# NVlabs/nvdiffrecmc

Measured on NVIDIA H100. Metric: shadow_rays_per_second_train_step, higher is better.
Workload: dtype f32

## Files before the change

include/mcshade.h:

```cpp
#ifndef MCSHADE_H
#define MCSHADE_H
#include <stdint.h>

#ifdef __cplusplus
extern "C" {
#endif

#define MCS_ABI_VERSION 2

typedef struct mcs_tensor {
    const void *ptr;
    int32_t sizes[4];
    int32_t strides[4];
} mcs_tensor;

typedef struct mcs_ctx mcs_ctx;
typedef void *mcs_stream;

int mcs_abi_version(void);
const char *mcs_last_error(void);

int mcs_ctx_create(mcs_ctx **out);
int mcs_ctx_destroy(mcs_ctx *ctx);

int mcs_bvh_build(mcs_ctx *ctx, const float *verts, int32_t V, const int32_t *tris, int32_t T, uint32_t rebuild, mcs_stream stream);

int mcs_bvh_export(mcs_ctx *ctx, uint32_t *morton, int32_t *prim, int32_t *left, int32_t *right, float *lo, float *hi, mcs_stream stream);

int mcs_trace_visibility(mcs_ctx *ctx, const float *ro, const float *rd, int64_t n, uint8_t *vis, mcs_stream stream);

int mcs_trace_closest(mcs_ctx *ctx, const float *ro, const float *rd, int64_t n, int32_t *tri_id, float *tuv, mcs_stream stream);

int mcs_env_shade_fwd(mcs_ctx *ctx,
                      const mcs_tensor *mask, const mcs_tensor *ro, const mcs_tensor *gb_pos, const mcs_tensor *gb_normal,
                      const mcs_tensor *gb_view_pos, const mcs_tensor *gb_kd, const mcs_tensor *gb_ks,
                      const mcs_tensor *light, const mcs_tensor *pdf, const mcs_tensor *rows, const mcs_tensor *cols,
                      const mcs_tensor *perms,
                      uint32_t bsdf, uint32_t n_samples_x, uint32_t rnd_seed, const uint32_t *seed_offset_dev, float shadow_scale, int32_t batch_offset,
                      float *diff, float *spec, uint32_t *hit_record, uint32_t *rec_count, float *rec_rays, int32_t rec_slots, mcs_stream stream);

int mcs_env_shade_bwd(mcs_ctx *ctx,
                      const mcs_tensor *mask, const mcs_tensor *ro, const mcs_tensor *gb_pos, const mcs_tensor *gb_normal,
// ... 101 lines not shown
```

nvdiffrecmc_b200/_lib.py:

```python
import collections
import ctypes as C
import os
import subprocess
import sys
from concurrent.futures import ThreadPoolExecutor

_PKG = os.path.dirname(os.path.abspath(__file__))
_CSRC = os.path.join(_PKG, "csrc")
_LIBDIR = os.path.join(_PKG, "lib")
LIB_PATH = os.environ.get("MCS_LIB", os.path.join(_LIBDIR, "libmcshade.so"))
SOURCES = ["core.cu", "elementwise.cu", "denoise.cu", "bvh.cu", "envshade.cu", "lossmesh.cu", "light.cu", "raster.cu"]
NVCC_FLAGS = ["-O3", "-std=c++17", "-gencode", "arch=compute_90a,code=sm_90a", "-lineinfo", "-Xcompiler", "-fPIC"]


def _nvcc():
    for cand in (os.environ.get("CUDA_HOME", "") + "/bin/nvcc", "/usr/local/cuda/bin/nvcc", "nvcc"):
        if cand and (os.path.isabs(cand) and os.path.exists(cand)):
            return cand
    return "nvcc"


def build(force=False, verbose=False):
    os.makedirs(_LIBDIR, exist_ok=True)
    objdir = os.path.join(_LIBDIR, "obj")
# ... 31 lines not shown

class mcs_tensor(C.Structure):
    _fields_ = [("ptr", C.c_void_p), ("sizes", C.c_int32 * 4), ("strides", C.c_int32 * 4)]


_lib = None
_T = C.POINTER(mcs_tensor)
_P = C.c_void_p
_SIGS = {
    "mcs_abi_version": ([], C.c_int),
    "mcs_last_error": ([], C.c_char_p),
    "mcs_ctx_create": ([C.POINTER(_P)], C.c_int),
    "mcs_ctx_destroy": ([_P], C.c_int),
    "mcs_bvh_build": ([_P, _P, C.c_int32, _P, C.c_int32, C.c_uint32, _P], C.c_int),
    "mcs_bvh_export": ([_P] * 8, C.c_int),
    "mcs_trace_visibility": ([_P, _P, _P, C.c_int64, _P, _P], C.c_int),
    "mcs_trace_closest": ([_P, _P, _P, C.c_int64, _P, _P, _P], C.c_int),
    "mcs_env_shade_fwd": ([_P] + [_T] * 12 + [C.c_uint32, C.c_uint32, C.c_uint32, _P, C.c_float, C.c_int32, _P, _P, _P, _P, _P, C.c_int32, _P], C.c_int),
    "mcs_env_shade_bwd_replay": ([_T] * 6 + [C.c_uint32, C.c_uint32, C.c_float, _T, _T, _P, _P, C.c_int32] + [_P] * 6, C.c_int),
    "mcs_env_shade_records": ([_P] + [_T] * 12 + [C.c_uint32, C.c_uint32, C.c_uint32, _P, C.c_float, C.c_int32, _P, _P, _P, _P, _P], C.c_int),
    "mcs_env_shade_bwd": ([_P] + [_T] * 12 + [C.c_uint32, C.c_uint32, C.c_uint32, _P, C.c_float, C.c_int32, _T, _T] + [_P] * 7, C.c_int),
    "mcs_bilateral_fwd": ([_T, _T, _T, C.c_float, _P, _P], C.c_int),
    "mcs_bilateral_bwd": ([_T, _T, C.c_float, _T, _P, _P], C.c_int),
    "mcs_bilateral_fwd2": ([_T, _T, _T, _T, C.c_float, _P, _P, _P], C.c_int),
    "mcs_bilateral_bwd2": ([_T, _T, C.c_float, _T, _T, _P, _P, _P], C.c_int),
    "mcs_lambert_fwd": ([_T] * 2 + [_P] * 2, C.c_int),
    "mcs_lambert_bwd": ([_T] * 3 + [_P] * 3, C.c_int),
    "mcs_frostbite_fwd": ([_T] * 4 + [_P] * 2, C.c_int),
    "mcs_frostbite_bwd": ([_T] * 5 + [_P] * 5, C.c_int),
    "mcs_fresnel_shlick_fwd": ([_T] * 3 + [_P] * 2, C.c_int),
# ... 41 lines not shown
        raise RuntimeError(
            "libmcshade.so not found at %s -- build it with `python -c 'import __graft_entry__ as g; g.build()'` "
            "(nvcc, sm_90a). There is no CPU / PyTorch fallback for the hot path." % LIB_PATH)
    l = C.CDLL(LIB_PATH)
    for name, (args, res) in _SIGS.items():
        fn = getattr(l, name)
        fn.argtypes = args
        fn.restype = res
    if l.mcs_abi_version() != 2:
        raise RuntimeError("libmcshade ABI version mismatch")
    _lib = l
    return l


LAUNCHES = collections.Counter()
_KERNELS_PER_CALL = {"optix_build_bvh": 11, "bvh_export": 0, "update_pdf": 2, "rasterize": 2, "antialias_topology": 2}


def check(status, what):
    LAUNCHES[what] += _KERNELS_PER_CALL.get(what, 1)
    if status != 0:
        msg = lib().mcs_last_error()
        raise RuntimeError("%s failed (status %d): %s" % (what, status, msg.decode() if msg else "?"))


def _desc(ptr, sizes, strides):
    t = mcs_tensor()
    t.ptr = ptr
    for i in range(4):
        t.sizes[i] = int(sizes[i])
        t.strides[i] = int(strides[i])
# ... 45 lines not shown
```

nvdiffrecmc_b200/csrc/bvh.cu:

```cuda
#include "bvh_traverse.cuh"
#include "ctx.h"

int mcs_buf_reserve(DevBuf &b, size_t bytes, cudaStream_t s)
{
    if (bytes <= b.cap) return 0;
    size_t ncap = b.cap ? b.cap : 256;
    while (ncap < bytes) ncap *= 2;
    if (b.p) MCS_CUDA(cudaFreeAsync(b.p, s));
    b.p = nullptr; b.cap = 0;
    MCS_CUDA(cudaMallocAsync(&b.p, ncap, s));
    b.cap = ncap;
    return 0;
}

namespace {

__device__ __forceinline__ uint32_t f2ord(float f) { uint32_t b = __float_as_uint(f); return (b & 0x80000000u) ? ~b : (b | 0x80000000u); }
__device__ __forceinline__ float ord2f(uint32_t u) { return __uint_as_float((u & 0x80000000u) ? (u & 0x7FFFFFFFu) : ~u); }

__global__ void k_bounds_init(uint32_t *bounds)
{
    int i = threadIdx.x;
    if (i < 12) bounds[i] = ((i / 3) & 1) ? 0u : 0xFFFFFFFFu;
}
// ... 303 lines not shown
            nodes[1] = make_float4(INFINITY, -INFINITY, INFINITY, -INFINITY);
            nodes[2] = make_float4(lo[2], hi[2], INFINITY, -INFINITY);
            nodes[3] = make_float4(__int_as_float(~((0 << 3) | (T - 1))), __int_as_float(~0), 0.0f, 0.0f);
        }
        return;
    }
    if (i >= T - 1) return;
    int c0 = left[i], c1 = right[i];
    const float *l0 = lo + 3 * (size_t)c0, *h0 = hi + 3 * (size_t)c0, *l1 = lo + 3 * (size_t)c1, *h1 = hi + 3 * (size_t)c1;
    nodes[4 * (size_t)i + 0] = make_float4(l0[0], h0[0], l0[1], h0[1]);
    nodes[4 * (size_t)i + 1] = make_float4(l1[0], h1[0], l1[1], h1[1]);
    nodes[4 * (size_t)i + 2] = make_float4(l0[2], h0[2], l1[2], h1[2]);
    nodes[4 * (size_t)i + 3] = make_float4(__int_as_float(child_code(c0, T, range)), __int_as_float(child_code(c1, T, range)), 0.0f, 0.0f);
}

__device__ __forceinline__ void emit_nodeq(const int i, int T, const int32_t *left, const int32_t *right, const int2 *range, const float *lo, const float *hi,
                                           uint4 *nodesq4, float *qgrid)
{
    float org[3], inv_cell[3];
#pragma unroll
    for (int a = 0; a < 3; ++a) {
        org[a] = lo[a];
        const float ext = __fsub_rn(hi[a], lo[a]);
        int e;
        const float m = frexpf(fmaxf(ext, 1e-30f) * (1.0f / 65532.0f), &e);
        const int k = (m == 0.5f) ? e - 1 : e;
        inv_cell[a] = ldexpf(1.0f, -k);
        if (i == 0) { qgrid[a] = org[a]; qgrid[3 + a] = ldexpf(1.0f, k); qgrid[6 + a] = inv_cell[a]; }
    }
    const bool tiny = T <= MCS_LEAF_MAX;
    if (tiny ? i != 0 : i >= T - 1) return;
    int cn[2], code[2];
    if (tiny) { cn[0] = 0; cn[1] = -1; code[0] = ~((0 << 3) | (T - 1)); code[1] = ~0; }
    else { cn[0] = left[i]; cn[1] = right[i]; code[0] = child_code(cn[0], T, range); code[1] = child_code(cn[1], T, range); }
    int gn[4] = {-1, -1, -1, -1}, gcode[4] = {~0, ~0, ~0, ~0}, ng = 0;
#pragma unroll
    for (int c = 0; c < 2; ++c) {
        if (cn[c] < 0) continue;
        if (code[c] < 0) { gn[ng] = cn[c]; gcode[ng] = code[c]; ++ng; }
        else {
            const int g0 = left[cn[c]], g1 = right[cn[c]];
            gn[ng] = g0; gcode[ng] = child_code(g0, T, range); ++ng;
            gn[ng] = g1; gcode[ng] = child_code(g1, T, range); ++ng;
        }
    }
    uint32_t leaf_bits = 0u;
#pragma unroll
    for (int c = 0; c < 4; ++c) leaf_bits |= (gcode[c] < 0 ? 1u : 0u) << c;
#pragma unroll
    for (int c = 0; c < 4; ++c) {
        uint32_t ql[3] = {65535u, 65535u, 65535u}, qh[3] = {0u, 0u, 0u};
        if (gn[c] >= 0) {
#pragma unroll
            for (int a = 0; a < 3; ++a) {
                const float fl = floorf(__fmul_rn(__fsub_rn(lo[3 * (size_t)gn[c] + a], org[a]), inv_cell[a])) - 2.0f;
                const float fh = ceilf(__fmul_rn(__fsub_rn(hi[3 * (size_t)gn[c] + a], org[a]), inv_cell[a])) + 2.0f;
                ql[a] = (uint32_t)fminf(fmaxf(fl, 0.0f), 65535.0f);
                qh[a] = (uint32_t)fminf(fmaxf(fh, 0.0f), 65535.0f);
            }
        }
        const uint32_t payload = (uint32_t)(gcode[c] < 0 ? ~gcode[c] : gcode[c]) & 0x0FFFFFFFu;
        nodesq4[4 * (size_t)i + c] = make_uint4(ql[0] | (qh[0] << 16), ql[1] | (qh[1] << 16), ql[2] | (qh[2] << 16), payload | (c == 0 ? leaf_bits << 28 : 0u));
    }
}

__global__ void __launch_bounds__(256) k_emit_both(int T, const int32_t *left, const int32_t *right, const int2 *range, const float *lo, const float *hi,
                                                   float4 *nodes, uint4 *nodesq4, float *qgrid)
{
    const int i = blockIdx.x * blockDim.x + threadIdx.x;
    emit_node(i, T, left, right, range, lo, hi, nodes);
    emit_nodeq(i, T, left, right, range, lo, hi, nodesq4, qgrid);
}

typedef BvhView VisView;
__global__ void __launch_bounds__(128) k_visibility(VisView b, const float *__restrict__ ro, const float *__restrict__ rd, int64_t n, uint8_t *__restrict__ vis)
{
    int64_t i = (int64_t)blockIdx.x * blockDim.x + threadIdx.x;
    if (i >= n) return;
    f3 o = F3(ro[3 * i], ro[3 * i + 1], ro[3 * i + 2]), d = F3(rd[3 * i], rd[3 * i + 1], rd[3 * i + 2]);
    vis[i] = bvh_occluded(b, o, d) ? 0 : 1;
}

__global__ void __launch_bounds__(128) k_closest(BvhView b, const float *__restrict__ ro, const float *__restrict__ rd, int64_t n,
                                                 int32_t *__restrict__ tri_id, float *__restrict__ tuv)
{
    int64_t i = (int64_t)blockIdx.x * blockDim.x + threadIdx.x;
// ... 14 lines not shown
{
    MCS_REQUIRE(out != nullptr, "mcs_ctx_create: null output pointer");
    int dev = 0;
    MCS_CUDA(cudaGetDevice(&dev));
    mcs_ctx *c = new mcs_ctx();
    c->device = dev;
    *out = c;
    return 0;
}

int mcs_ctx_destroy(mcs_ctx *c)
{
    if (!c) return 0;
    DevBuf *bufs[] = {&c->bounds, &c->tlo, &c->thi, &c->keys, &c->keys_alt, &c->vals, &c->vals_alt, &c->left, &c->right, &c->parent,
                      &c->lo, &c->hi, &c->flags, &c->range, &c->sort_tmp, &c->nodes, &c->tris, &c->nodesq4, &c->qgrid, &c->lcg_skip[0], &c->lcg_skip[1], &c->lcg_skip[2], &c->lcg_skip[3],
                      &c->counters, &c->mtx_inv};
    for (DevBuf *b : bufs)
        if (b->p) cudaFree(b->p);
    delete c;
    return 0;
}

int mcs_bvh_build(mcs_ctx *c, const float *verts, int32_t V, const int32_t *tris, int32_t T, uint32_t rebuild, mcs_stream stream)
{
    cudaStream_t s = (cudaStream_t)stream;
    MCS_REQUIRE(c != nullptr, "mcs_bvh_build: null context");
    MCS_REQUIRE(verts && tris, "mcs_bvh_build: null geometry pointer");
    MCS_REQUIRE(T > 0 && V > 0, "Got empty training triangle mesh (unrecoverable discontinuity)");
    MCS_REQUIRE(T <= (1 << 25), "mcs_bvh_build: at most 2^25 triangles (28-bit child words of the quantised nodes), got %d", T);
    MCS_REQUIRE(rebuild != 0 || c->T == T, "mcs_bvh_build: refit (rebuild=0) needs an existing structure with the same triangle count (have %d, got %d)", c->T, T);
    const size_t nT = (size_t)T, nN = 2 * nT - 1;
// ... 24 lines not shown
    if (rebuild) {
        k_morton<<<nblk(T, 256), 256, 0, s>>>(tlo, thi, T, bounds, (uint32_t *)c->keys_alt.p, (int32_t *)c->vals_alt.p);
        MCS_LAUNCH_CHECK();
        if (int e = rs_sort_pairs((uint32_t *)c->keys_alt.p, (int32_t *)c->vals_alt.p, (uint32_t *)c->keys.p, (int32_t *)c->vals.p, T, c->sort_tmp, s)) return e;
        if (T > 1) {
            k_karras<<<nblk(T - 1, 256), 256, 0, s>>>((const uint32_t *)c->keys_alt.p, T, (int32_t *)c->left.p, (int32_t *)c->right.p, (int32_t *)c->parent.p,
                                                      (int2 *)c->range.p);
            MCS_LAUNCH_CHECK();
        }
    }
    MCS_CUDA(cudaMemsetAsync(c->flags.p, 0, nT * sizeof(int), s));
    k_leaves_refit<<<nblk(T, REFIT_THREADS), REFIT_THREADS, 0, s>>>(verts, tris, T, tlo, thi, (const int32_t *)c->vals_alt.p, bounds, (const int32_t *)c->left.p,
                                                                   (const int32_t *)c->right.p, (const int32_t *)c->parent.p, (const int2 *)c->range.p,
                                                                   (float *)c->lo.p, (float *)c->hi.p, (int *)c->flags.p, (float4 *)c->tris.p);
    MCS_LAUNCH_CHECK();
    k_emit_both<<<nblk(T > 1 ? T - 1 : 1, 256), 256, 0, s>>>(T, (const int32_t *)c->left.p, (const int32_t *)c->right.p, (const int2 *)c->range.p,
                                                              (const float *)c->lo.p, (const float *)c->hi.p, (float4 *)c->nodes.p, (uint4 *)c->nodesq4.p,
                                                              (float *)c->qgrid.p);
    MCS_LAUNCH_CHECK();
    c->T = T; c->V = V;
    return 0;
}

int mcs_bvh_export(mcs_ctx *c, uint32_t *morton, int32_t *prim, int32_t *left, int32_t *right, float *lo, float *hi, mcs_stream stream)
{
    cudaStream_t s = (cudaStream_t)stream;
    MCS_REQUIRE(c && c->T > 0, "mcs_bvh_export: no acceleration structure built");
    size_t T = (size_t)c->T;
    MCS_CUDA(cudaMemcpyAsync(morton, c->keys_alt.p, T * sizeof(uint32_t), cudaMemcpyDeviceToDevice, s));
    MCS_CUDA(cudaMemcpyAsync(prim, c->vals_alt.p, T * sizeof(int32_t), cudaMemcpyDeviceToDevice, s));
    if (T > 1) {
        MCS_CUDA(cudaMemcpyAsync(left, c->left.p, (T - 1) * sizeof(int32_t), cudaMemcpyDeviceToDevice, s));
        MCS_CUDA(cudaMemcpyAsync(right, c->right.p, (T - 1) * sizeof(int32_t), cudaMemcpyDeviceToDevice, s));
    }
    MCS_CUDA(cudaMemcpyAsync(lo, c->lo.p, (2 * T - 1) * 3 * sizeof(float), cudaMemcpyDeviceToDevice, s));
    MCS_CUDA(cudaMemcpyAsync(hi, c->hi.p, (2 * T - 1) * 3 * sizeof(float), cudaMemcpyDeviceToDevice, s));
    return 0;
}

int mcs_trace_visibility(mcs_ctx *c, const float *ro, const float *rd, int64_t n, uint8_t *vis, mcs_stream stream)
{
    MCS_REQUIRE(c && c->T > 0, "mcs_trace_visibility: no acceleration structure built (call mcs_bvh_build first)");
    MCS_REQUIRE(n >= 0 && (n == 0 || (ro && rd && vis)), "mcs_trace_visibility: bad arguments");
    if (n == 0) return 0;
    VisView b{(const float4 *)c->nodes.p, (const float4 *)c->tris.p, nullptr, nullptr};
    k_visibility<<<nblk(n, 128), 128, 0, (cudaStream_t)stream>>>(b, ro, rd, n, vis);
    MCS_LAUNCH_CHECK();
    return 0;
}

int mcs_trace_closest(mcs_ctx *c, const float *ro, const float *rd, int64_t n, int32_t *tri_id, float *tuv, mcs_stream stream)
{
    MCS_REQUIRE(c && c->T > 0, "mcs_trace_closest: no acceleration structure built (call mcs_bvh_build first)");
    MCS_REQUIRE(n >= 0 && (n == 0 || (ro && rd && tri_id && tuv)), "mcs_trace_closest: bad arguments");
// ... 9 lines not shown
```

nvdiffrecmc_b200/csrc/ctx.h:

```cpp
#pragma once
#include "common.cuh"

#define MCS_SKIP_TABLES 4
#define MCS_COUNTER_RING 64

struct DevBuf {
    void *p = nullptr;
    size_t cap = 0;
};

struct mcs_ctx {
    int device = 0;
    int T = 0, V = 0;
    DevBuf bounds;
    DevBuf tlo, thi;
    DevBuf keys, keys_alt;
    DevBuf vals, vals_alt;
    DevBuf left, right, parent;
    DevBuf lo, hi;
    DevBuf flags;
    DevBuf range;
    DevBuf sort_tmp;
    DevBuf nodes;
    DevBuf tris;
    DevBuf nodesq4;
    DevBuf qgrid;
    DevBuf lcg_skip[MCS_SKIP_TABLES];
    int skip_N[MCS_SKIP_TABLES] = {0, 0, 0, 0};
    int n_skip = 0;
    unsigned skip_evict = 0;
    DevBuf counters;
    unsigned counter_next = 0;
    DevBuf mtx_inv;
};

int mcs_buf_reserve(DevBuf &b, size_t bytes, cudaStream_t s);
```

nvdiffrecmc_b200/csrc/envshade.cu:

```cuda
#include "bsdf.cuh"
#include "bvh_traverse.cuh"
#include "ctx.h"
#include "exact.cuh"
#include <vector>

namespace {

constexpr float MIN_ROUGHNESS = 0.08f;

struct EnvParams {
    TView mask, ro, pos, nrm, view, kd, ks;
    const float *light; int l_s1, l_s2, l_s3;
    const float *pdf; int p_s1, p_s2;
    const float *rows; int r_s;
    const float *cols; int c_s1, c_s2;
    const int32_t *perms; int pm_s1, pm_s3; uint32_t n_perms;
    int Hl, Wl, m_rows, m_cols;
    int B, H, W;
    int N, S;
    uint32_t bsdf, seed;
    const uint32_t *seed_dev;
    int batch_offset;
    float shadow_scale;
    BvhView bvh;
// ... 195 lines not shown
#ifndef MCS_SPLIT_WALKS
#define MCS_SPLIT_WALKS 1
#endif
#ifndef MCS_SPLIT_BELOW
#define MCS_SPLIT_BELOW 20
#endif
#ifndef MCS_QSTACK
#define MCS_QSTACK 100
#endif
#ifndef MCS_LEAF_BATCH
#define MCS_LEAF_BATCH 32
#endif
#ifndef MCS_REFILL_BELOW
#define MCS_REFILL_BELOW 24
#endif
constexpr int NW = MCS_CTA_WARPS;
constexpr int SEG = 128;
constexpr int QTOT = NW * SEG;
#ifndef MCS_PCAP
#define MCS_PCAP 160
#endif
constexpr int PCAP = MCS_PCAP;
constexpr int PIXRING = 256;
static_assert(QTOT <= 65536, "queue entry index is stored in 16 bits");
static_assert(SEG <= 256 && SEG % 32 == 0, "sample slot within a fill is stored in 8 bits");

struct BlockQueue {
    float dx[QTOT], dy[QTOT], dz[QTOT], mis[QTOT];
    uint32_t tex[QTOT];
    uint16_t vlist[QTOT];
// ... 184 lines not shown

__device__ __forceinline__ void trace_queue(const EnvParams &p, BlockQueue &q, const int warp, const int lane)
{
    constexpr int REFILL_BELOW = MCS_REFILL_BELOW;
    constexpr int LEAF_BATCH = MCS_LEAF_BATCH;
    unsigned lt;
    asm("mov.u32 %0, %%lanemask_lt;" : "=r"(lt));
    int pend = 0;
    int my = -1;
    int node = 0, sp = 0, sb = 0;
    int stack[MCS_QSTACK];
    RayQ r; r.ax = r.ay = r.az = 1.0f; r.bx = r.by = r.bz = 0.0f; r.nx = r.ny = r.nz = 0x7410u; r.fx = r.fy = r.fz = 0x7432u;
    const BvhView b = p.bvh;
    uint2 *pl = q.pl[warp];
    int seg = warp, exhausted = 0;

    auto leaf_batch = [&](int n) {
        __syncwarp();
        const int base = pend - n;
        if (lane < n) {
            const uint2 ent = pl[base + lane];
            const int e = (int)ent.x;
            if (!(q.tex[e] >> 31)) {
                const int code = (int)ent.y;
                const int start = code >> 3, cnt = (code & 7) + 1;
                const int ps = e / SEG;
                const f3 o = F3(q.ro[ps][0], q.ro[ps][1], q.ro[ps][2]);
                const f3 d = F3(q.dx[e], q.dy[e], q.dz[e]);
                bool hit = false;
                for (int k = 0; k < cnt && !hit; ++k) {
                    const float4 *t = b.tris + 3 * (size_t)(start + k);
                    const float4 t0 = __ldg(t), t1 = __ldg(t + 1), t2 = __ldg(t + 2);
                    float tt, uu, vv;
                    hit = mt_hit(o, d, F3(t0.x, t0.y, t0.z), F3(t1.x, t1.y, t1.z), F3(t2.x, t2.y, t2.z), MCS_TMAX, tt, uu, vv);
                }
                if (hit) atomicOr(&q.tex[e], 0x80000000u);
            }
        }
        pend = base;
        __syncwarp();
    };

    while (true) {
        unsigned idle = __ballot_sync(0xFFFFFFFFu, my < 0);
        while (idle && exhausted < NW) {
            const int need = __popc(idle);
            int base = 0;
            if (lane == 0) base = atomicAdd(&q.seg_head[seg], need);
            base = __shfl_sync(0xFFFFFFFFu, base, 0);
            const int avail = q.seg_cnt[seg] - base;
            if (avail <= 0) { seg = seg + 1 == NW ? 0 : seg + 1; ++exhausted; continue; }
            const int take = avail < need ? avail : need;
            const int rank = __popc(idle & lt);
            if (my < 0 && rank < take) {
                const int idx = seg * SEG + base + rank;
                my = idx;
                r = rayq_fetch(b.qgrid, q.rog[seg], q.dx[idx], q.dy[idx], q.dz[idx]);
                node = 0; sp = 0; sb = 0;
            }
            if (take < need) { seg = seg + 1 == NW ? 0 : seg + 1; ++exhausted; }
            idle = __ballot_sync(0xFFFFFFFFu, my < 0);
        }
#if MCS_SPLIT_WALKS
        if (exhausted >= NW && idle) {
            const unsigned donors = __ballot_sync(0xFFFFFFFFu, my >= 0 && sp > sb);
            if (donors) {
                const int npair = min(__popc(idle), __popc(donors));
                uint2 *xch = pl + (PCAP - 32);
                const int kd = __popc(donors & lt), ki = __popc(idle & lt);
                if (my >= 0 && sp > sb && kd < npair) { xch[kd] = make_uint2((unsigned)my, (unsigned)stack[sb]); ++sb; }
                __syncwarp();
                if (my < 0 && ki < npair) {
                    const uint2 g = xch[ki];
// ... 5 lines not shown
            }
        }
#endif
        int nact = __popc(__ballot_sync(0xFFFFFFFFu, my >= 0));
        if (nact == 0) {
            if (pend == 0) break;
            leaf_batch(pend < 32 ? pend : 32);
            continue;
        }
        const int thresh = exhausted < NW ? REFILL_BELOW : (MCS_SPLIT_WALKS ? MCS_SPLIT_BELOW : 1);
        do {
            const int cur = my;
            unsigned lmask = 0u;
            int c0 = 0, c1 = 0, c2 = 0, c3 = 0;
            if (my >= 0) {
                const uint4 *n = b.nodesq4 + 4 * (size_t)node;
                const uint4 k0 = __ldg(n), k1 = __ldg(n + 1), k2 = __ldg(n + 2), k3 = __ldg(n + 3);
                const bool h0 = qslab(k0, r), h1 = qslab(k1, r), h2 = qslab(k2, r), h3 = qslab(k3, r);
                const unsigned hm = (h0 ? 1u : 0u) | (h1 ? 2u : 0u) | (h2 ? 4u : 0u) | (h3 ? 8u : 0u);
                const unsigned lb = k0.w >> 28;
                c0 = (int)(k0.w & 0x0FFFFFFFu); c1 = (int)k1.w; c2 = (int)k2.w; c3 = (int)k3.w;
                lmask = hm & lb;
                const unsigned im = hm & ~lb;
                stack[sp] = c0; sp += (int)(im & 1u);
                stack[sp] = c1; sp += (int)((im >> 1) & 1u);
                stack[sp] = c2; sp += (int)((im >> 2) & 1u);
                stack[sp] = c3; sp += (int)(im >> 3);
                if (im) { node = (im & 8u) ? c3 : ((im & 4u) ? c2 : ((im & 2u) ? c1 : c0)); --sp; }
                else if (sp > sb) node = stack[--sp];
                else my = -1;
// ... 1 lines not shown
            for (unsigned mL = __ballot_sync(0xFFFFFFFFu, lmask != 0u); mL; mL = __ballot_sync(0xFFFFFFFFu, lmask != 0u)) {
                if (lmask) {
                    const unsigned low = lmask & (0u - lmask);
                    const int code = (low & 3u) ? ((low & 1u) ? c0 : c1) : ((low & 4u) ? c2 : c3);
                    pl[pend + __popc(mL & lt)] = make_uint2((unsigned)cur, (unsigned)code);
                    lmask ^= low;
                }
                pend += __popc(mL);
                if (PCAP < 160 && pend >= LEAF_BATCH) leaf_batch(32);
            }
            nact = __popc(__ballot_sync(0xFFFFFFFFu, my >= 0));
        } while (pend < LEAF_BATCH && nact >= thresh);
        while (pend >= LEAF_BATCH) leaf_batch(32);
        if (my >= 0 && (q.tex[my] >> 31)) my = -1;
    }
    __syncwarp();
}

template <int MODE>
__global__ void __launch_bounds__(NW * 32, 32 / NW) env_shade_kernel(const EnvParams p)
{
    extern __shared__ __align__(16) unsigned char smem_raw[];
    const int lane = threadIdx.x & 31, warp = threadIdx.x >> 5;
    BlockQueue &q = *reinterpret_cast<BlockQueue *>(smem_raw);
    BlockQueueRec *qr = MODE == 2 ? reinterpret_cast<BlockQueueRec *>(smem_raw + sizeof(BlockQueue)) : nullptr;

    const int64_t npix = (int64_t)p.B * p.H * p.W;
    const unsigned int nchunks = (unsigned int)((npix + 31) / 32);
    const int S = p.S, items = 2 * S;
    const float sample_frac = (xf(1.0f) / xf((float)(unsigned)(p.N * p.N))).v;
// ... 342 lines not shown
    p.Hl = light->sizes[1]; p.Wl = light->sizes[2];
    MCS_REQUIRE(light->sizes[3] == 3 && p.Hl >= 2 && p.Wl >= 2, "env_shade: light must be [Hl>=2, Wl>=2, 3]");
    MCS_REQUIRE(p.Hl < 32768 && p.Wl < 65536, "env_shade: light probe too large");
    MCS_REQUIRE(pdf->sizes[1] == p.Hl && pdf->sizes[2] == p.Wl && cols->sizes[1] == p.Hl && cols->sizes[2] == p.Wl && rows->sizes[1] == p.Hl,
                "env_shade: pdf / rows / cols do not match the light probe resolution");
    p.light = (const float *)light->ptr; p.l_s1 = light->strides[1]; p.l_s2 = light->strides[2]; p.l_s3 = light->strides[3];
    p.pdf = (const float *)pdf->ptr; p.p_s1 = pdf->strides[1]; p.p_s2 = pdf->strides[2];
    p.rows = (const float *)rows->ptr; p.r_s = rows->strides[1];
    p.cols = (const float *)cols->ptr; p.c_s1 = cols->strides[1]; p.c_s2 = cols->strides[2];
    p.N = (int)n_samples_x; p.S = p.N * p.N;
    p.hit_words = (2 * p.S + 31) / 32;
    MCS_REQUIRE(perms->sizes[3] == p.S && perms->sizes[1] >= 1, "env_shade: perms must be [P, n_samples_x^2]");
    p.perms = (const int32_t *)perms->ptr; p.pm_s1 = perms->strides[1]; p.pm_s3 = perms->strides[3]; p.n_perms = (uint32_t)perms->sizes[1];
    p.m_rows = cdf_iters(p.Hl); p.m_cols = cdf_iters(p.Wl);
    p.bsdf = bsdf; p.seed = rnd_seed; p.seed_dev = seed_offset_dev; p.batch_offset = batch_offset; p.shadow_scale = shadow_scale;
    p.bvh = BvhView{(const float4 *)ctx->nodes.p, (const float4 *)ctx->tris.p, (const float *)ctx->qgrid.p, (const uint4 *)ctx->nodesq4.p};
    if (int e = ensure_skip_table(ctx, p.N, s, &p.skip)) return e;
    if (int e = mcs_buf_reserve(ctx->counters, MCS_COUNTER_RING * 64, s)) return e;
    p.chunk_counter = (unsigned int *)((char *)ctx->counters.p + 64 * (size_t)(ctx->counter_next++ % MCS_COUNTER_RING));
    MCS_CUDA(cudaMemsetAsync(p.chunk_counter, 0, sizeof(unsigned int), s));
    return 0;
}

template <int MODE>
static int launch_env(const EnvParams &p, cudaStream_t s)
{
    int dev = 0, sms = 0, per_sm = 0;
    MCS_CUDA(cudaGetDevice(&dev));
    MCS_CUDA(cudaDeviceGetAttribute(&sms, cudaDevAttrMultiProcessorCount, dev));
    const size_t smem = sizeof(BlockQueue) + (MODE == 2 ? sizeof(BlockQueueRec) : 0);
    MCS_CUDA(cudaFuncSetAttribute(env_shade_kernel<MODE>, cudaFuncAttributeMaxDynamicSharedMemorySize, (int)smem));
// ... 101 lines not shown
    p.sample_frac = 1.0f / (float)(n_samples_x * n_samples_x);
    p.pos_grad = gb_pos_grad; p.nrm_grad = gb_normal_grad; p.kd_grad = gb_kd_grad; p.ks_grad = gb_ks_grad; p.light_grad = light_grad;
    MCS_CUDA(cudaMemsetAsync(light_grad, 0, sizeof(float) * 3 * (size_t)p.Hl * p.Wl, s));
    int dev = 0, sms = 0;
    MCS_CUDA(cudaGetDevice(&dev));
    MCS_CUDA(cudaDeviceGetAttribute(&sms, cudaDevAttrMultiProcessorCount, dev));
    const int64_t npix = (int64_t)p.B * p.H * p.W;
    int64_t want = (npix + 255) / 256;
    int grid = (int)(want < (int64_t)sms * 8 ? want : (int64_t)sms * 8);
    if (grid < 1) grid = 1;
    env_shade_replay_kernel<<<grid, 256, 0, s>>>(p);
    MCS_LAUNCH_CHECK();
    return 0;
}

}
```

nvdiffrecmc_b200/optixutils/ops.py:

```python
import ctypes as C

import numpy as np
import torch

from .. import _lib as L

_BSDF_MODES = ['pbr', 'diffuse', 'white']
HIT_RECORD_REPLAY = "rays"
RAY_RECORD_MAX_BYTES = 32 << 30
RAY_RECORD_MAX_FREE_FRACTION = 0.5


_fits_cache = {}


def _ray_record_fits(nbytes, device):
    if nbytes > RAY_RECORD_MAX_BYTES:
        return False
    key = (str(device), int(nbytes))
    if torch.cuda.is_current_stream_capturing():
        return _fits_cache.get(key, True)
    _fits_cache[key] = _ray_record_fits_now(nbytes, device)
    return _fits_cache[key]

# ... 186 lines not shown
                                      L.stream_ptr()), "trace_closest")
    return tid, tuv


def bvh_export(optix_ctx):
    T = optix_ctx._geom[1].shape[0]
    dev = optix_ctx._geom[0].device
    morton = torch.empty(T, dtype=torch.int32, device=dev); prim = torch.empty(T, dtype=torch.int32, device=dev)
    left = torch.empty(max(T - 1, 1), dtype=torch.int32, device=dev); right = torch.empty(max(T - 1, 1), dtype=torch.int32, device=dev)
    lo = torch.empty(2 * T - 1, 3, dtype=torch.float32, device=dev); hi = torch.empty(2 * T - 1, 3, dtype=torch.float32, device=dev)
    L.check(L.lib().mcs_bvh_export(optix_ctx.cpp_wrapper, morton.data_ptr(), prim.data_ptr(), left.data_ptr(), right.data_ptr(), lo.data_ptr(),
                                   hi.data_ptr(), L.stream_ptr()), "bvh_export")
    return dict(morton=morton, prim=prim, left=left[:T - 1], right=right[:T - 1], lo=lo, hi=hi)


class _bilateral_denoiser_func(torch.autograd.Function):
    @staticmethod
    def forward(ctx, col, nrm, zdz, sigma):
        L.require_cuda(col, nrm, zdz)
        ctx.save_for_backward(nrm, zdz)
        ctx.sigma = sigma
        B, H, W = col.shape[0], col.shape[1], col.shape[2]
        out = torch.empty(B, H, W, 4, dtype=torch.float32, device=col.device)
        c, n, z = L.nhwc(_f32(col, "col")), L.nhwc(_f32(nrm, "nrm")), L.nhwc(_f32(zdz, "zdz"))
        L.check(L.lib().mcs_bilateral_fwd(C.byref(c), C.byref(n), C.byref(z), float(sigma), out.data_ptr(), L.stream_ptr()), "bilateral_denoiser (forward)")
        return out

    @staticmethod
    def backward(ctx, out_grad):
        nrm, zdz = ctx.saved_tensors
# ... 81 lines not shown
```

Baseline: 5341.

## Build SAH-aware PLOC BVH with multi-triangle leaves for shadow traversal

For meshes up to a size limit, adds a single-block PLOC agglomerative clustering pass that builds a binary BVH with SAH-based leaf collapsing (up to 8 triangles per leaf). It then emits a 4-wide quantized node array and reorders triangles so leaves are contiguous. The shadow-ray tracer in the shading kernel uses these reordered triangles, aiming to reduce node visits and triangle tests compared with the LBVH. The cost is two extra kernels per BVH build, and k_ploc runs on only one CTA, which may be slow for larger meshes. Optional traversal counters and an export function are also added.

```diff
diff --git a/include/mcshade.h b/include/mcshade.h
--- a/include/mcshade.h
+++ b/include/mcshade.h
@@ -26,6 +26,8 @@
 int mcs_bvh_build(mcs_ctx *ctx, const float *verts, int32_t V, const int32_t *tris, int32_t T, uint32_t rebuild, mcs_stream stream);
 
 int mcs_bvh_export(mcs_ctx *ctx, uint32_t *morton, int32_t *prim, int32_t *left, int32_t *right, float *lo, float *hi, mcs_stream stream);
+
+int mcs_bvh_export_shadow(mcs_ctx *ctx, uint32_t *nodesq4, float *tris, float *qgrid, mcs_stream stream);
 
 int mcs_trace_visibility(mcs_ctx *ctx, const float *ro, const float *rd, int64_t n, uint8_t *vis, mcs_stream stream);
 
diff --git a/nvdiffrecmc_b200/_lib.py b/nvdiffrecmc_b200/_lib.py
--- a/nvdiffrecmc_b200/_lib.py
+++ b/nvdiffrecmc_b200/_lib.py
@@ -69,6 +69,7 @@
     "mcs_ctx_destroy": ([_P], C.c_int),
     "mcs_bvh_build": ([_P, _P, C.c_int32, _P, C.c_int32, C.c_uint32, _P], C.c_int),
     "mcs_bvh_export": ([_P] * 8, C.c_int),
+    "mcs_bvh_export_shadow": ([_P] * 5, C.c_int),
     "mcs_trace_visibility": ([_P, _P, _P, C.c_int64, _P, _P], C.c_int),
     "mcs_trace_closest": ([_P, _P, _P, C.c_int64, _P, _P, _P], C.c_int),
     "mcs_env_shade_fwd": ([_P] + [_T] * 12 + [C.c_uint32, C.c_uint32, C.c_uint32, _P, C.c_float, C.c_int32, _P, _P, _P, _P, _P, C.c_int32, _P], C.c_int),
@@ -140,7 +141,7 @@
 
 
 LAUNCHES = collections.Counter()
-_KERNELS_PER_CALL = {"optix_build_bvh": 11, "bvh_export": 0, "update_pdf": 2, "rasterize": 2, "antialias_topology": 2}
+_KERNELS_PER_CALL = {"optix_build_bvh": 13, "bvh_export": 0, "bvh_export_shadow": 0, "update_pdf": 2, "rasterize": 2, "antialias_topology": 2}
 
 
 def check(status, what):
diff --git a/nvdiffrecmc_b200/csrc/bvh.cu b/nvdiffrecmc_b200/csrc/bvh.cu
--- a/nvdiffrecmc_b200/csrc/bvh.cu
+++ b/nvdiffrecmc_b200/csrc/bvh.cu
@@ -341,10 +341,8 @@
     nodes[4 * (size_t)i + 3] = make_float4(__int_as_float(child_code(c0, T, range)), __int_as_float(child_code(c1, T, range)), 0.0f, 0.0f);
 }
 
-__device__ __forceinline__ void emit_nodeq(const int i, int T, const int32_t *left, const int32_t *right, const int2 *range, const float *lo, const float *hi,
-                                           uint4 *nodesq4, float *qgrid)
-{
-    float org[3], inv_cell[3];
+__device__ __forceinline__ void quant_grid(const float *lo, const float *hi, float org[3], float inv_cell[3], float cell[3])
+{
 #pragma unroll
     for (int a = 0; a < 3; ++a) {
         org[a] = lo[a];
@@ -353,10 +351,34 @@
         const float m = frexpf(fmaxf(ext, 1e-30f) * (1.0f / 65532.0f), &e);
         const int k = (m == 0.5f) ? e - 1 : e;
         inv_cell[a] = ldexpf(1.0f, -k);
-        if (i == 0) { qgrid[a] = org[a]; qgrid[3 + a] = ldexpf(1.0f, k); qgrid[6 + a] = inv_cell[a]; }
-    }
+        cell[a] = ldexpf(1.0f, k);
+    }
+}
+
+__device__ __forceinline__ uint4 quant_child(const float *l, const float *h, const float org[3], const float inv_cell[3], uint32_t word)
+{
+    uint32_t ql[3] = {65535u, 65535u, 65535u}, qh[3] = {0u, 0u, 0u};
+    if (l) {
+#pragma unroll
+        for (int a = 0; a < 3; ++a) {
+            const float fl = floorf(__fmul_rn(__fsub_rn(l[a], org[a]), inv_cell[a])) - 2.0f;
+            const float fh = ceilf(__fmul_rn(__fsub_rn(h[a], org[a]), inv_cell[a])) + 2.0f;
+            ql[a] = (uint32_t)fminf(fmaxf(fl, 0.0f), 65535.0f);
+            qh[a] = (uint32_t)fminf(fmaxf(fh, 0.0f), 65535.0f);
+        }
+    }
+    return make_uint4(ql[0] | (qh[0] << 16), ql[1] | (qh[1] << 16), ql[2] | (qh[2] << 16), word);
+}
+
+__device__ __forceinline__ void emit_nodeq(const int i, int T, const int32_t *left, const int32_t *right, const int2 *range, const float *lo, const float *hi,
+                                           uint4 *nodesq4, float *qgrid)
+{
+    float org[3], inv_cell[3], cell[3];
+    quant_grid(lo, hi, org, inv_cell, cell);
+    if (i == 0)
+        for (int a = 0; a < 3; ++a) { qgrid[a] = org[a]; qgrid[3 + a] = cell[a]; qgrid[6 + a] = inv_cell[a]; }
     const bool tiny = T <= MCS_LEAF_MAX;
-    if (tiny ? i != 0 : i >= T - 1) return;
+    if (!nodesq4 || (tiny ? i != 0 : i >= T - 1)) return;
     int cn[2], code[2];
     if (tiny) { cn[0] = 0; cn[1] = -1; code[0] = ~((0 << 3) | (T - 1)); code[1] = ~0; }
     else { cn[0] = left[i]; cn[1] = right[i]; code[0] = child_code(cn[0], T, range); code[1] = child_code(cn[1], T, range); }
@@ -376,18 +398,10 @@
     for (int c = 0; c < 4; ++c) leaf_bits |= (gcode[c] < 0 ? 1u : 0u) << c;
 #pragma unroll
     for (int c = 0; c < 4; ++c) {
-        uint32_t ql[3] = {65535u, 65535u, 65535u}, qh[3] = {0u, 0u, 0u};
-        if (gn[c] >= 0) {
-#pragma unroll
-            for (int a = 0; a < 3; ++a) {
-                const float fl = floorf(__fmul_rn(__fsub_rn(lo[3 * (size_t)gn[c] + a], org[a]), inv_cell[a])) - 2.0f;
-                const float fh = ceilf(__fmul_rn(__fsub_rn(hi[3 * (size_t)gn[c] + a], org[a]), inv_cell[a])) + 2.0f;
-                ql[a] = (uint32_t)fminf(fmaxf(fl, 0.0f), 65535.0f);
-                qh[a] = (uint32_t)fminf(fmaxf(fh, 0.0f), 65535.0f);
-            }
-        }
         const uint32_t payload = (uint32_t)(gcode[c] < 0 ? ~gcode[c] : gcode[c]) & 0x0FFFFFFFu;
-        nodesq4[4 * (size_t)i + c] = make_uint4(ql[0] | (qh[0] << 16), ql[1] | (qh[1] << 16), ql[2] | (qh[2] << 16), payload | (c == 0 ? leaf_bits << 28 : 0u));
+        const bool used = gn[c] >= 0;
+        nodesq4[4 * (size_t)i + c] = quant_child(used ? lo + 3 * (size_t)gn[c] : nullptr, used ? hi + 3 * (size_t)gn[c] : nullptr, org, inv_cell,
+                                                 payload | (c == 0 ? leaf_bits << 28 : 0u));
     }
 }
 
@@ -397,6 +411,181 @@
     const int i = blockIdx.x * blockDim.x + threadIdx.x;
     emit_node(i, T, left, right, range, lo, hi, nodes);
     emit_nodeq(i, T, left, right, range, lo, hi, nodesq4, qgrid);
+}
+
+#ifndef MCS_SAH_MAX_TRIS
+#define MCS_SAH_MAX_TRIS 16384
+#endif
+#define PLOC_THREADS 1024
+#define PLOC_RADIUS 8
+#define SAH_LEAF_MAX 8
+#define SAH_CI 1.2f
+#define SAH_CT 1.0f
+
+__device__ __forceinline__ float half_area(float4 l, float4 h)
+{
+    const float dx = h.x - l.x, dy = h.y - l.y, dz = h.z - l.z;
+    return dx * dy + dy * dz + dz * dx;
+}
+
+__device__ __forceinline__ int2 block_exscan2(int2 v, int2 *total, int2 *sw)
+{
+    const int lane = threadIdx.x & 31, warp = threadIdx.x >> 5;
+    int2 x = v;
+#pragma unroll
+    for (int o = 1; o < 32; o <<= 1) {
+        const int yx = __shfl_up_sync(0xFFFFFFFFu, x.x, o), yy = __shfl_up_sync(0xFFFFFFFFu, x.y, o);
+        if (lane >= o) { x.x += yx; x.y += yy; }
+    }
+    if (lane == 31) sw[warp] = x;
+    __syncthreads();
+    if (warp == 0) {
+        int2 w = sw[lane];
+#pragma unroll
+        for (int o = 1; o < 32; o <<= 1) {
+            const int yx = __shfl_up_sync(0xFFFFFFFFu, w.x, o), yy = __shfl_up_sync(0xFFFFFFFFu, w.y, o);
+            if (lane >= o) { w.x += yx; w.y += yy; }
+        }
+        sw[lane] = w;
+    }
+    __syncthreads();
+    const int2 base = warp ? sw[warp - 1] : make_int2(0, 0);
+    *total = sw[31];
+    return make_int2(base.x + x.x - v.x, base.y + x.y - v.y);
+}
+
+struct ShadowTree {
+    int32_t *left, *right;
+    float4 *box;
+    int32_t *cnt;
+    int32_t *first;
+};
+
+__global__ void __launch_bounds__(PLOC_THREADS) k_ploc(int T, const float *lo, const float *hi, ShadowTree st, int32_t *cid, float4 *cbox, int32_t *nn,
+                                                       int32_t *round_id)
+{
+    __shared__ int2 sw[32];
+    const int tid = threadIdx.x;
+    for (int j = tid; j < T; j += PLOC_THREADS) {
+        const size_t n = (size_t)(T - 1 + j);
+        const float4 l = make_float4(lo[3 * n], lo[3 * n + 1], lo[3 * n + 2], 0.0f), h = make_float4(hi[3 * n], hi[3 * n + 1], hi[3 * n + 2], 0.0f);
+        cid[j] = T - 1 + j;
+        cbox[2 * j] = make_float4(l.x, l.y, l.z, SAH_CT * half_area(l, h));
+        cbox[2 * j + 1] = make_float4(h.x, h.y, h.z, __int_as_float(1));
+    }
+    __syncthreads();
+    int n = T, next_id = T - 2, rounds = 0, buf = 0;
+    while (n > 1) {
+        int32_t *ci = cid + (size_t)buf * T, *co = cid + (size_t)(buf ^ 1) * T;
+        float4 *bi = cbox + (size_t)buf * 2 * T, *bo = cbox + (size_t)(buf ^ 1) * 2 * T;
+        if (tid == 0) round_id[rounds] = next_id;
+        for (int i = tid; i < n; i += PLOC_THREADS) {
+            const float4 li = bi[2 * i], hi_ = bi[2 * i + 1];
+            float best = INFINITY;
+            int bj = -1;
+            const int j0 = max(0, i - PLOC_RADIUS), j1 = min(n - 1, i + PLOC_RADIUS);
+            for (int j = j0; j <= j1; ++j) {
+                if (j == i) continue;
+                const float4 lj = bi[2 * j], hj = bi[2 * j + 1];
+                const float a = fminf(half_area(make_float4(fminf(li.x, lj.x), fminf(li.y, lj.y), fminf(li.z, lj.z), 0.0f),
+                                                make_float4(fmaxf(hi_.x, hj.x), fmaxf(hi_.y, hj.y), fmaxf(hi_.z, hj.z), 0.0f)), INFINITY);
+                if (a < best || bj < 0) { best = a; bj = j; }
+            }
+            nn[i] = bj;
+        }
+        __syncthreads();
+        const int per = (n + PLOC_THREADS - 1) / PLOC_THREADS, beg = min(n, tid * per), end = min(n, beg + per);
+        int2 mine = make_int2(0, 0);
+        for (int i = beg; i < end; ++i) {
+            const int j = nn[i];
+            const bool mutual = nn[j] == i;
+            mine.x += (!mutual || i < j) ? 1 : 0;
+            mine.y += (mutual && i < j) ? 1 : 0;
+        }
+        int2 tot;
+        int2 pos = block_exscan2(mine, &tot, sw);
+        for (int i = beg; i < end; ++i) {
+            const int j = nn[i];
+            const bool mutual = nn[j] == i;
+            if (mutual && i > j) continue;
+            if (!mutual) { co[pos.x] = ci[i]; bo[2 * pos.x] = bi[2 * i]; bo[2 * pos.x + 1] = bi[2 * i + 1]; ++pos.x; continue; }
+            const float4 la = bi[2 * i], ha = bi[2 * i + 1], lb = bi[2 * j], hb = bi[2 * j + 1];
+            const float4 l = make_float4(fminf(la.x, lb.x), fminf(la.y, lb.y), fminf(la.z, lb.z), 0.0f);
+            const float4 h = make_float4(fmaxf(ha.x, hb.x), fmaxf(ha.y, hb.y), fmaxf(ha.z, hb.z), 0.0f);
+            const float A = half_area(l, h);
+            const int cnt = __float_as_int(ha.w) + __float_as_int(hb.w);
+            const float c_int = SAH_CI * A + la.w + lb.w, c_leaf = SAH_CT * A * (float)cnt;
+            const bool leaf = cnt <= SAH_LEAF_MAX && c_leaf <= c_int;
+            const int id = next_id - pos.y;
+            st.left[id] = ci[i]; st.right[id] = ci[j];
+            st.box[2 * id] = l; st.box[2 * id + 1] = h;
+            st.cnt[id] = leaf ? -cnt : cnt;
+            co[pos.x] = id;
+            bo[2 * pos.x] = make_float4(l.x, l.y, l.z, leaf ? c_leaf : c_int);
+            bo[2 * pos.x + 1] = make_float4(h.x, h.y, h.z, __int_as_float(cnt));
+            ++pos.x; ++pos.y;
+        }
+        n = tot.x; next_id -= tot.y; buf ^= 1; ++rounds;
+        __syncthreads();
+    }
+    if (tid == 0) { round_id[rounds] = next_id; st.first[0] = 0; }
+    __syncthreads();
+    for (int r = rounds - 1; r >= 0; --r) {
+        for (int id = round_id[r + 1] + 1 + tid; id <= round_id[r]; id += PLOC_THREADS) {
+            const int f = st.first[id], l = st.left[id];
+            st.first[l] = f;
+            st.first[st.right[id]] = f + (l >= T - 1 ? 1 : abs(st.cnt[l]));
+        }
+        __syncthreads();
+    }
+}
+
+__global__ void __launch_bounds__(256) k_emit_shadow(int T, ShadowTree st, const float *lo, const float *hi, const float4 *__restrict__ tris,
+                                                     float4 *__restrict__ stris, uint4 *__restrict__ nodesq4)
+{
+    const int i = blockIdx.x * blockDim.x + threadIdx.x;
+    if (i >= T) return;
+    {
+        const int d = st.first[T - 1 + i];
+        stris[3 * (size_t)d] = tris[3 * (size_t)i];
+        stris[3 * (size_t)d + 1] = tris[3 * (size_t)i + 1];
+        stris[3 * (size_t)d + 2] = tris[3 * (size_t)i + 2];
+    }
+    if (i >= T - 1 || (i != 0 && st.cnt[i] < 0)) return;
+    auto is_node = [&](int x) { return x < T - 1 && st.cnt[x] > 0; };
+    int s[4] = {st.left[i], st.right[i], -1, -1}, ns = 2;
+    while (ns < 4) {
+        int b = -1;
+        float ba = -1.0f;
+        for (int c = 0; c < ns; ++c)
+            if (is_node(s[c])) {
+                const float a = half_area(st.box[2 * s[c]], st.box[2 * s[c] + 1]);
+                if (a > ba) { ba = a; b = c; }
+            }
+        if (b < 0) break;
+        const int x = s[b];
+        s[b] = st.left[x]; s[ns++] = st.right[x];
+    }
+    float org[3], inv_cell[3], cell[3];
+    quant_grid(lo, hi, org, inv_cell, cell);
+    uint32_t leaf_bits = 0u;
+    for (int c = 0; c < 4; ++c) leaf_bits |= (c >= ns || !is_node(s[c]) ? 1u : 0u) << c;
+    for (int c = 0; c < 4; ++c) {
+        uint32_t payload = 0u;
+        const float *l = nullptr, *h = nullptr;
+        float bl[3], bh[3];
+        if (c < ns) {
+            const int x = s[c];
+            if (x >= T - 1) { l = lo + 3 * (size_t)x; h = hi + 3 * (size_t)x; payload = (uint32_t)st.first[x] << 3; }
+            else {
+                const float4 a = st.box[2 * x], b = st.box[2 * x + 1];
+                bl[0] = a.x; bl[1] = a.y; bl[2] = a.z; bh[0] = b.x; bh[1] = b.y; bh[2] = b.z;
+                l = bl; h = bh;
+                payload = st.cnt[x] > 0 ? (uint32_t)x : ((uint32_t)st.first[x] << 3) | (uint32_t)(-st.cnt[x] - 1);
+            }
+        }
+        nodesq4[4 * (size_t)i + c] = quant_child(l, h, org, inv_cell, (payload & 0x0FFFFFFFu) | (c == 0 ? leaf_bits << 28 : 0u));
+    }
 }
 
 typedef BvhView VisView;
@@ -441,7 +630,7 @@
     if (!c) return 0;
     DevBuf *bufs[] = {&c->bounds, &c->tlo, &c->thi, &c->keys, &c->keys_alt, &c->vals, &c->vals_alt, &c->left, &c->right, &c->parent,
                       &c->lo, &c->hi, &c->flags, &c->range, &c->sort_tmp, &c->nodes, &c->tris, &c->nodesq4, &c->qgrid, &c->lcg_skip[0], &c->lcg_skip[1], &c->lcg_skip[2], &c->lcg_skip[3],
-                      &c->counters, &c->mtx_inv};
+                      &c->counters, &c->mtx_inv, &c->sleft, &c->sright, &c->scnt, &c->sbox, &c->sfirst, &c->swork, &c->stris};
     for (DevBuf *b : bufs)
         if (b->p) cudaFree(b->p);
     delete c;
@@ -496,10 +685,29 @@
                                                                    (const int32_t *)c->right.p, (const int32_t *)c->parent.p, (const int2 *)c->range.p,
                                                                    (float *)c->lo.p, (float *)c->hi.p, (int *)c->flags.p, (float4 *)c->tris.p);
     MCS_LAUNCH_CHECK();
+    const bool sah = T > MCS_LEAF_MAX && T <= MCS_SAH_MAX_TRIS;
     k_emit_both<<<nblk(T > 1 ? T - 1 : 1, 256), 256, 0, s>>>(T, (const int32_t *)c->left.p, (const int32_t *)c->right.p, (const int2 *)c->range.p,
-                                                              (const float *)c->lo.p, (const float *)c->hi.p, (float4 *)c->nodes.p, (uint4 *)c->nodesq4.p,
-                                                              (float *)c->qgrid.p);
+                                                              (const float *)c->lo.p, (const float *)c->hi.p, (float4 *)c->nodes.p,
+                                                              sah ? nullptr : (uint4 *)c->nodesq4.p, (float *)c->qgrid.p);
     MCS_LAUNCH_CHECK();
+    if (sah) {
+        if (int e = mcs_buf_reserve(c->sleft, nT * sizeof(int32_t), s)) return e;
+        if (int e = mcs_buf_reserve(c->sright, nT * sizeof(int32_t), s)) return e;
+        if (int e = mcs_buf_reserve(c->scnt, nT * sizeof(int32_t), s)) return e;
+        if (int e = mcs_buf_reserve(c->sbox, nT * 2 * sizeof(float4), s)) return e;
+        if (int e = mcs_buf_reserve(c->sfirst, nN * sizeof(int32_t), s)) return e;
+        if (int e = mcs_buf_reserve(c->swork, nT * (4 * sizeof(float4) + 4 * sizeof(int32_t)), s)) return e;
+        if (int e = mcs_buf_reserve(c->stris, nT * 3 * sizeof(float4), s)) return e;
+        const ShadowTree st{(int32_t *)c->sleft.p, (int32_t *)c->sright.p, (float4 *)c->sbox.p, (int32_t *)c->scnt.p, (int32_t *)c->sfirst.p};
+        float4 *cbox = (float4 *)c->swork.p;
+        int32_t *cid = (int32_t *)(cbox + 4 * nT);
+        k_ploc<<<1, PLOC_THREADS, 0, s>>>(T, (const float *)c->lo.p, (const float *)c->hi.p, st, cid, cbox, cid + 2 * nT, cid + 3 * nT);
+        MCS_LAUNCH_CHECK();
+        k_emit_shadow<<<nblk(T, 256), 256, 0, s>>>(T, st, (const float *)c->lo.p, (const float *)c->hi.p, (const float4 *)c->tris.p, (float4 *)c->stris.p,
+                                                   (uint4 *)c->nodesq4.p);
+        MCS_LAUNCH_CHECK();
+    }
+    c->shadow_sah = sah;
     c->T = T; c->V = V;
     return 0;
 }
@@ -520,6 +728,17 @@
     return 0;
 }
 
+int mcs_bvh_export_shadow(mcs_ctx *c, uint32_t *nodesq4, float *tris, float *qgrid, mcs_stream stream)
+{
+    cudaStream_t s = (cudaStream_t)stream;
+    MCS_REQUIRE(c && c->T > 0, "mcs_bvh_export_shadow: no acceleration structure built");
+    const size_t T = (size_t)c->T;
+    MCS_CUDA(cudaMemcpyAsync(nodesq4, c->nodesq4.p, (T > 1 ? T - 1 : 1) * 4 * sizeof(uint4), cudaMemcpyDeviceToDevice, s));
+    MCS_CUDA(cudaMemcpyAsync(tris, c->shadow_sah ? c->stris.p : c->tris.p, T * 3 * sizeof(float4), cudaMemcpyDeviceToDevice, s));
+    MCS_CUDA(cudaMemcpyAsync(qgrid, c->qgrid.p, 9 * sizeof(float), cudaMemcpyDeviceToDevice, s));
+    return 0;
+}
+
 int mcs_trace_visibility(mcs_ctx *c, const float *ro, const float *rd, int64_t n, uint8_t *vis, mcs_stream stream)
 {
     MCS_REQUIRE(c && c->T > 0, "mcs_trace_visibility: no acceleration structure built (call mcs_bvh_build first)");
diff --git a/nvdiffrecmc_b200/csrc/ctx.h b/nvdiffrecmc_b200/csrc/ctx.h
--- a/nvdiffrecmc_b200/csrc/ctx.h
+++ b/nvdiffrecmc_b200/csrc/ctx.h
@@ -25,6 +25,12 @@
     DevBuf tris;
     DevBuf nodesq4;
     DevBuf qgrid;
+    bool shadow_sah = false;
+    DevBuf sleft, sright, scnt;
+    DevBuf sbox;
+    DevBuf sfirst;
+    DevBuf swork;
+    DevBuf stris;
     DevBuf lcg_skip[MCS_SKIP_TABLES];
     int skip_N[MCS_SKIP_TABLES] = {0, 0, 0, 0};
     int n_skip = 0;
diff --git a/nvdiffrecmc_b200/csrc/envshade.cu b/nvdiffrecmc_b200/csrc/envshade.cu
--- a/nvdiffrecmc_b200/csrc/envshade.cu
+++ b/nvdiffrecmc_b200/csrc/envshade.cu
@@ -233,6 +233,12 @@
 #ifndef MCS_REFILL_BELOW
 #define MCS_REFILL_BELOW 24
 #endif
+#ifndef MCS_COUNT_TRAVERSAL
+#define MCS_COUNT_TRAVERSAL 0
+#endif
+#if MCS_COUNT_TRAVERSAL
+__device__ unsigned long long g_trace_counts[3];
+#endif
 constexpr int NW = MCS_CTA_WARPS;
 constexpr int SEG = 128;
 constexpr int QTOT = NW * SEG;
@@ -447,6 +453,9 @@
     const BvhView b = p.bvh;
     uint2 *pl = q.pl[warp];
     int seg = warp, exhausted = 0;
+#if MCS_COUNT_TRAVERSAL
+    unsigned long long n_rays = 0, n_visits = 0, n_tests = 0;
+#endif
 
     auto leaf_batch = [&](int n) {
         __syncwarp();
@@ -462,6 +471,9 @@
                 const f3 d = F3(q.dx[e], q.dy[e], q.dz[e]);
                 bool hit = false;
                 for (int k = 0; k < cnt && !hit; ++k) {
+#if MCS_COUNT_TRAVERSAL
+                    ++n_tests;
+#endif
                     const float4 *t = b.tris + 3 * (size_t)(start + k);
                     const float4 t0 = __ldg(t), t1 = __ldg(t + 1), t2 = __ldg(t + 2);
                     float tt, uu, vv;
@@ -490,6 +502,9 @@
                 my = idx;
                 r = rayq_fetch(b.qgrid, q.rog[seg], q.dx[idx], q.dy[idx], q.dz[idx]);
                 node = 0; sp = 0; sb = 0;
+#if MCS_COUNT_TRAVERSAL
+                ++n_rays;
+#endif
             }
             if (take < need) { seg = seg + 1 == NW ? 0 : seg + 1; ++exhausted; }
             idle = __ballot_sync(0xFFFFFFFFu, my < 0);
@@ -525,6 +540,9 @@
             unsigned lmask = 0u;
             int c0 = 0, c1 = 0, c2 = 0, c3 = 0;
             if (my >= 0) {
+#if MCS_COUNT_TRAVERSAL
+                ++n_visits;
+#endif
                 const uint4 *n = b.nodesq4 + 4 * (size_t)node;
                 const uint4 k0 = __ldg(n), k1 = __ldg(n + 1), k2 = __ldg(n + 2), k3 = __ldg(n + 3);
                 const bool h0 = qslab(k0, r), h1 = qslab(k1, r), h2 = qslab(k2, r), h3 = qslab(k3, r);
@@ -556,6 +574,9 @@
         while (pend >= LEAF_BATCH) leaf_batch(32);
         if (my >= 0 && (q.tex[my] >> 31)) my = -1;
     }
+#if MCS_COUNT_TRAVERSAL
+    atomicAdd(&g_trace_counts[0], n_rays); atomicAdd(&g_trace_counts[1], n_visits); atomicAdd(&g_trace_counts[2], n_tests);
+#endif
     __syncwarp();
 }
 
@@ -928,7 +949,8 @@
     p.perms = (const int32_t *)perms->ptr; p.pm_s1 = perms->strides[1]; p.pm_s3 = perms->strides[3]; p.n_perms = (uint32_t)perms->sizes[1];
     p.m_rows = cdf_iters(p.Hl); p.m_cols = cdf_iters(p.Wl);
     p.bsdf = bsdf; p.seed = rnd_seed; p.seed_dev = seed_offset_dev; p.batch_offset = batch_offset; p.shadow_scale = shadow_scale;
-    p.bvh = BvhView{(const float4 *)ctx->nodes.p, (const float4 *)ctx->tris.p, (const float *)ctx->qgrid.p, (const uint4 *)ctx->nodesq4.p};
+    p.bvh = BvhView{(const float4 *)ctx->nodes.p, (const float4 *)(ctx->shadow_sah ? ctx->stris.p : ctx->tris.p), (const float *)ctx->qgrid.p,
+                    (const uint4 *)ctx->nodesq4.p};
     if (int e = ensure_skip_table(ctx, p.N, s, &p.skip)) return e;
     if (int e = mcs_buf_reserve(ctx->counters, MCS_COUNTER_RING * 64, s)) return e;
     p.chunk_counter = (unsigned int *)((char *)ctx->counters.p + 64 * (size_t)(ctx->counter_next++ % MCS_COUNTER_RING));
@@ -1060,4 +1082,17 @@
     return 0;
 }
 
-}
+#if MCS_COUNT_TRAVERSAL
+int mcs_trace_counts(unsigned long long *out, int reset)
+{
+    MCS_CUDA(cudaDeviceSynchronize());
+    MCS_CUDA(cudaMemcpyFromSymbol(out, g_trace_counts, sizeof(g_trace_counts)));
+    if (reset) {
+        const unsigned long long zero[3] = {0, 0, 0};
+        MCS_CUDA(cudaMemcpyToSymbol(g_trace_counts, zero, sizeof(zero)));
+    }
+    return 0;
+}
+#endif
+
+}
diff --git a/nvdiffrecmc_b200/optixutils/ops.py b/nvdiffrecmc_b200/optixutils/ops.py
--- a/nvdiffrecmc_b200/optixutils/ops.py
+++ b/nvdiffrecmc_b200/optixutils/ops.py
@@ -224,6 +224,16 @@
     return dict(morton=morton, prim=prim, left=left[:T - 1], right=right[:T - 1], lo=lo, hi=hi)
 
 
+def bvh_export_shadow(optix_ctx):
+    T = optix_ctx._geom[1].shape[0]
+    dev = optix_ctx._geom[0].device
+    nodes = torch.empty(max(T - 1, 1), 4, 4, dtype=torch.int32, device=dev)
+    tris = torch.empty(T, 3, 4, dtype=torch.float32, device=dev)
+    qgrid = torch.empty(9, dtype=torch.float32, device=dev)
+    L.check(L.lib().mcs_bvh_export_shadow(optix_ctx.cpp_wrapper, nodes.data_ptr(), tris.data_ptr(), qgrid.data_ptr(), L.stream_ptr()), "bvh_export_shadow")
+    return dict(nodes=nodes, tris=tris, qgrid=qgrid)
+
+
 class _bilateral_denoiser_func(torch.autograd.Function):
     @staticmethod
     def forward(ctx, col, nrm, zdz, sigma):
```

After: 5520, median of 6. +3.3%, better.
